# mikostrzewa/AprilSLAM

Measured on AMD Instinct MI355X. Metric: frames/sec at 1280x720, 20 tags/frame (detection + batched PnP), higher is better.
Workload: dtype u8/f64

## Files before the change

### aprilslam_amd/_lib.py

```python
import ctypes as C
import os

import numpy as np

_HERE = os.path.dirname(os.path.abspath(__file__))
LIB_PATH = os.environ.get("ASL_LIB") or os.path.join(_HERE, "libaprilslam.so")


class AslError(RuntimeError):
    pass


class AslDetection(C.Structure):
    _fields_ = [("id", C.c_int32), ("hamming", C.c_int32), ("margin", C.c_float), ("frame", C.c_int32),
                ("center", C.c_double * 2), ("corners", (C.c_double * 2) * 4)]


class AslPose(C.Structure):
    _fields_ = [("rvec", C.c_double * 3), ("tvec", C.c_double * 3), ("T", C.c_double * 16), ("ok", C.c_int32),
                ("reserved", C.c_int32)]


class AslMapTag(C.Structure):
    _fields_ = [("T", C.c_double * 12), ("valid", C.c_int32), ("reserved", C.c_int32)]
# ... 418 lines not shown
                                   corners.ctypes.data_as(dp), Kc.ctypes.data_as(dp), float(tag_size), int(fixed_tag),
                                   cam.ctypes.data_as(dp), tag.ctypes.data_as(dp), int(iters), stats.ctypes.data_as(dp)))
        return cam.reshape(-1, 4, 4), tag.reshape(-1, 4, 4), stats

    def debug_counters(self):
        buf = np.zeros(18, dtype=np.int64)
        n = C.c_size_t()
        check(self._L.asl_debug_fetch(self._h, 5, buf.ctypes.data, buf.nbytes, C.byref(n)))
        return buf

    def debug_image(self, what):
        c = self.debug_counters()
        B, sw, sh = int(c[0]), int(c[1]), int(c[2])
        dt = np.uint8 if what in (0, 1) else np.uint32
        buf = np.zeros((B, sh, sw), dtype=dt)
        n = C.c_size_t()
        check(self._L.asl_debug_fetch(self._h, what, buf.ctypes.data, buf.nbytes, C.byref(n)))
        return buf

    def debug_quads(self, cap=65536):
        buf = np.zeros(cap, dtype=QUAD_DTYPE)
        n = C.c_size_t()
        check(self._L.asl_debug_fetch(self._h, 4, buf.ctypes.data, buf.nbytes, C.byref(n)))
        return buf[:n.value]

    def debug_clusters(self):
        ncl = int(self.debug_counters()[3])
        buf = np.zeros((max(ncl, 1), 3), dtype=np.uint64)
        n = C.c_size_t()
        check(self._L.asl_debug_fetch(self._h, 6, buf.ctypes.data, buf.nbytes, C.byref(n)))
        return buf[:n.value]

    def debug_refit(self, reps):
        buf = np.zeros(7, dtype=np.int64)
        n = C.c_size_t()
        check(self._L.asl_debug_fetch(self._h, 7, buf.ctypes.data, int(reps), C.byref(n)))
        return buf

    def debug_division_check(self, exponent_limit=100):
        buf = np.zeros(2, dtype=np.int64)
        n = C.c_size_t()
        check(self._L.asl_debug_fetch(self._h, 8, buf.ctypes.data, int(exponent_limit), C.byref(n)))
        return int(buf[0]), int(buf[1])

    def phase_cycles(self, reset=True):
        buf = (C.c_uint64 * 64)()
        check(self._L.asl_debug_phase_cycles(self._h, buf, 1 if reset else 0))
        return np.array(list(buf), dtype=np.uint64)

    def set_profiling(self, on=True):
        check(self._L.asl_set_profiling(self._h, 1 if on else 0))

    def stage_times(self):
        names = (C.c_char_p * 32)()
        ms = (C.c_float * 32)()
        n = C.c_int()
        check(self._L.asl_stage_times(self._h, names, ms, 32, C.byref(n)))
        return {names[i].decode(): float(ms[i]) for i in range(n.value)}
```

### aprilslam_amd/csrc/aprilslam.hip

```cpp
#include "../../include/aprilslam.h"

#include <algorithm>
#include <chrono>
#include <cmath>
#include <cstdarg>
#include <cstdio>
#include <cstring>
#include <string>
#include <vector>

#include "asl_common.h"
#include "tag_standard41h12.inc"

#include "k_threshold.inc"
#include "k_cc.inc"
#include "k_cluster.inc"
#include "k_seg.inc"
#include "k_xchg.inc"
#include "k_quad.inc"
#include "k_decode.inc"
#include "k_pnp.inc"
#include "k_dedup.inc"
#include "k_graph.inc"
#include "k_render.inc"
// ... 181 lines not shown
    d->fam.width_at_border = kTag41h12WidthAtBorder;
    d->fam.total_width = kTag41h12TotalWidth;
    d->fam.reversed_border = 1;
    d->fam.ncodes = kTag41h12PinnedIds;
    for (int i = 0; i < kTag41h12NBits; i++) { d->fam.bit_x[i] = kTag41h12BitX[i]; d->fam.bit_y[i] = kTag41h12BitY[i]; }
    if (hipMalloc((void **)&d->d_codes, sizeof(unsigned long long) * kTag41h12NCodes) != hipSuccess) {
        delete d;
        return fail(ASL_ENOMEM, "hipMalloc(code book) failed");
    }
    if (hipMemcpy(d->d_codes, kTag41h12Codes, sizeof(unsigned long long) * kTag41h12NCodes, hipMemcpyHostToDevice) != hipSuccess) {
        (void)hipFree(d->d_codes);
        delete d;
        return fail(ASL_EDEVICE, "hipMemcpy(code book) failed");
    }
    d->fam.codes = d->d_codes;
    if (build_code_index(d)) {
        d->idx_start.release(); d->idx_entries.release();
        (void)hipFree(d->d_codes);
        delete d;
        return fail(ASL_ENOMEM, "code-book index allocation failed");
    }
    if (d->wtab.ensure(WEIGHT_TABLE_N)) {
        (void)hipFree(d->d_codes);
        delete d;
        return fail(ASL_ENOMEM, "hipMalloc(weight table) failed");
    }
    hipLaunchKernelGGL(k_weight_table, dim3((WEIGHT_TABLE_N + 255) / 256), dim3(256), 0, 0, d->wtab.p);
    if (hipDeviceSynchronize() != hipSuccess) {
        d->wtab.release();
        (void)hipFree(d->d_codes);
        delete d;
        return fail(ASL_EDEVICE, "weight table kernel failed");
    }
    (void)hipFuncSetAttribute(reinterpret_cast<const void *>(&k_fit_quads<256, true, CLASS3_CAP / 256>), hipFuncAttributeMaxDynamicSharedMemorySize, QUAD_LDS_BYTES(CLASS3_CAP));
    *out = d;
    return ASL_OK;
}

extern "C" void asl_detector_destroy(asl_detector *d)
{
    if (!d) return;
    (void)hipSetDevice(d->device);
    if (d->pending) (void)hipStreamSynchronize(d->p_stream);
    d->rootmask.release(); d->quad_list.release(); d->dense_tiles.release(); d->dense_seg.release(); d->seg_edges.release(); d->wmask.release(); d->bmask.release();
    d->dbg_thresh.release(); d->dbg_labels.release();
    d->frame_ndets.release(); d->frame_idx.release(); d->frame_nkeep.release(); d->frame_off.release(); d->out_det.release(); d->out_pose.release();
    if (d->host_pose) (void)hipHostFree(d->host_pose);
    if (d->host_nkeep) (void)hipHostFree(d->host_nkeep);
    d->in.release(); d->dgray.release(); d->tmin.release(); d->tmax.release(); d->tcut.release();
    d->parent.release(); d->sizes.release(); d->hkeys.release(); d->points.release(); d->hcounts.release(); d->class_lists.release(); d->stage_pos.release(); d->frame_cursor.release(); d->stage_rec.release();
    d->slot_cluster.release(); d->clusters.release(); d->quads.release(); d->scratch.release(); d->side_mom.release(); d->quadH.release(); d->wtab.release(); d->dets.release();
    d->counters.release(); d->pnp_corners.release(); d->pnp_out.release(); d->pnp_ok.release();
    d->gn.release();
    d->loc_obs.release(); d->loc_map.release(); d->loc_out.release();
    d->cal_ws.release(); d->cal_out.release();
    d->map_ws.release(); d->map_lm.release(); d->map_out.release();
    if (d->aux_stream) (void)hipStreamDestroy(d->aux_stream);
    if (d->copy_stream) (void)hipStreamDestroy(d->copy_stream);
    if (d->host_stream) (void)hipStreamDestroy(d->host_stream);
    for (hipEvent_t e : d->copy_done) (void)hipEventDestroy(e);
    if (d->d_codes) (void)hipFree(d->d_codes);
    d->idx_start.release(); d->idx_entries.release();
    if (d->host_det) (void)hipHostFree(d->host_det);
    if (d->pinned_counters) (void)hipHostFree(d->pinned_counters);
    for (int i = 0; i <= MAX_STAGES; i++) if (d->ev[i]) (void)hipEventDestroy(d->ev[i]);
    delete d;
}
// ... 111 lines not shown
    bad |= d->seg_edges.ensure(B * (size_t)seg_nwx(g) * (size_t)((g.sh + SEG_TH - 1) / SEG_TH));
    bad |= d->scratch.ensure((size_t)d->max_points * 8);
    bad |= d->dets.ensure(d->max_dets);
    bad |= d->frame_ndets.ensure(B);
    bad |= d->frame_nkeep.ensure(B);
    bad |= d->frame_off.ensure(B);
    bad |= d->frame_idx.ensure(B * (size_t)d->dets_per_frame);
    bad |= d->out_det.ensure(d->max_dets);
    bad |= d->out_pose.ensure(d->max_dets);
    bad |= d->counters.ensure(CNT__N);
    if (bad) return fail(ASL_ENOMEM, "device workspace allocation failed (%zu frames of %dx%d)", B, g.sw, g.sh);
    return ASL_OK;
}

#define STAGE(name)                                                        \
    do {                                                                   \
        if (d->profiling && d->nev < MAX_STAGES) {                         \
            d->stage_names[d->nev] = name;                                 \
            HIPCHK(hipEventRecord(d->ev[d->nev], st));                     \
            d->nev++;                                                      \
        }                                                                  \
    } while (0)

static void launch_fit_class(asl_detector *d, const Geom &g, int cls, unsigned int B, hipStream_t st)
{
    const int want_rev = d->fam.reversed_border ? 1 : 0, want_norm = d->fam.reversed_border ? 0 : 1;
    int tag_width = d->fam.width_at_border / g.f;
    if (tag_width < 3) tag_width = 3;
    const unsigned int qgrid = std::min<unsigned int>(d->max_clusters, std::max<unsigned int>(16384u, 32u * B));
    const unsigned int q2grid = std::min<unsigned int>(d->max_clusters, 2048u);
    const unsigned int *list = d->class_lists.p + (size_t)cls * d->max_clusters;
    switch (cls) {
    case 0:
        hipLaunchKernelGGL((k_fit_quads<64, true, CLASS0_CAP / 64>), dim3(qgrid), dim3(64), QUAD_LDS_BYTES(CLASS0_CAP), st, d->clusters.p, list, d->counters.p, 0,
                           d->max_clusters, CLASS0_CAP, d->points.p, d->dgray.p, g, tag_width, want_rev, want_norm, d->scratch.p, d->quads.p, d->wtab.p, d->side_mom.p);
        break;
    case 1:
        hipLaunchKernelGGL((k_fit_quads<128, true, CLASS1_CAP / 128>), dim3(qgrid), dim3(128), QUAD_LDS_BYTES(CLASS1_CAP), st, d->clusters.p, list, d->counters.p, 1,
                           d->max_clusters, CLASS1_CAP, d->points.p, d->dgray.p, g, tag_width, want_rev, want_norm, d->scratch.p, d->quads.p, d->wtab.p, d->side_mom.p);
        break;
    case 2:
        hipLaunchKernelGGL((k_fit_quads<256, true, CLASS2_CAP / 256>), dim3(q2grid), dim3(256), QUAD_LDS_BYTES(CLASS2_CAP), st, d->clusters.p, list, d->counters.p, 2,
                           d->max_clusters, CLASS2_CAP, d->points.p, d->dgray.p, g, tag_width, want_rev, want_norm, d->scratch.p, d->quads.p, d->wtab.p, d->side_mom.p);
        break;
    case 3:
        hipLaunchKernelGGL((k_fit_quads<256, true, CLASS3_CAP / 256>), dim3(q2grid), dim3(256), QUAD_LDS_BYTES(CLASS3_CAP), st, d->clusters.p, list, d->counters.p, 3,
                           d->max_clusters, CLASS3_CAP, d->points.p, d->dgray.p, g, tag_width, want_rev, want_norm, d->scratch.p, d->quads.p, d->wtab.p, d->side_mom.p);
        break;
    default:
        hipLaunchKernelGGL((k_fit_quads<256, false, 0>), dim3(q2grid), dim3(256), 0, st, d->clusters.p, list, d->counters.p, 4, d->max_clusters, 0, d->points.p,
                           d->dgray.p, g, tag_width, want_rev, want_norm, d->scratch.p, d->quads.p, d->wtab.p, d->side_mom.p);
        break;
    }
}

static void launch_quad_finish(asl_detector *d, const Geom &g, hipStream_t st)
{
    int tag_width = d->fam.width_at_border / g.f;
    if (tag_width < 3) tag_width = 3;
    hipLaunchKernelGGL(k_quad_finish, dim3(std::min<unsigned int>((d->max_clusters + 63) / 64, 4096u)), dim3(256), 0, st, d->quads.p, d->side_mom.p, d->counters.p,
                       d->max_clusters, tag_width);
}

static int enqueue_detect(asl_detector *d, const uint8_t *d_frames, const Geom &g, hipStream_t st, const CamDev *cam)
{
    dim3 blk(64, 4, 1);
    int thx = (g.sh + TILESZ - 1) / TILESZ;
    unsigned int B = (unsigned int)g.nframes;
    d->nev = 0;
    range_push("S0-S4 gray, decimate, threshold, segmentation, clusters");
    STAGE("k_hash_clear");
    hipLaunchKernelGGL(k_hash_clear, dim3((std::max<unsigned int>(d->nslots, std::max<unsigned int>(B, CNT__N)) + 255) / 256), dim3(256), 0, st, d->hkeys.p,
                       d->hcounts.p, d->nslots, d->counters.p, d->frame_cursor.p, d->frame_ndets.p, B);

    STAGE("k_decimate_minmax");
    if (g.f == 2) {
        const unsigned int ntile = (unsigned int)(g.tw * g.th);
        const unsigned int nrest = (unsigned int)(g.sw - 4 * g.tw) * (unsigned int)g.sh + (unsigned int)(g.sh - 4 * g.th) * (unsigned int)(4 * g.tw);
        if (ntile)
            hipLaunchKernelGGL((g.channels == 1 ? k_decimate2_tiles<1> : k_decimate2_tiles<3>), dim3((ntile + 255) / 256, B), dim3(256), 0, st, d_frames, g,
                               d->dgray.p, d->tmin.p, d->tmax.p);
        if (nrest)
            hipLaunchKernelGGL((g.channels == 1 ? k_decimate_rest<1> : k_decimate_rest<3>), dim3((nrest + 255) / 256, B), dim3(256), 0, st, d_frames, g,
// ... 14 lines not shown
        hipLaunchKernelGGL(k_seg_tile_dense, dim3(1024), dim3(64), 0, st, g, nwx, ntiles, d->wmask.p, d->bmask.p, d->parent.p, d->sizes.p,
                           d->rootmask.p, d->dense_seg.p, d->counters.p);
    }
    STAGE("k_seg_border");
    {
        const size_t nseams = nwx > 1 ? (size_t)B * g.sh * (nwx - 1) : 0;
        const unsigned int ncol_blocks = (unsigned int)((nseams + 63) / 64);
        const int nrb = (g.sh - 1) / SEG_TH;
        const unsigned int nrow_blocks = (unsigned int)nwx * (unsigned int)nrb * (unsigned int)B;
        if (ncol_blocks + nrow_blocks > 0)
            hipLaunchKernelGGL(k_seg_border, dim3(ncol_blocks + nrow_blocks), dim3(64), 0, st, d->wmask.p, d->bmask.p, d->seg_edges.p,
                               nwx * ((g.sh + SEG_TH - 1) / SEG_TH), g, nwx, d->parent.p, d->counters.p, ncol_blocks, nrb > 0 ? nrb : 1);
    }
    STAGE("k_seg_roots");
    hipLaunchKernelGGL(k_seg_roots, dim3((unsigned int)((nwords + 255) / 256)), dim3(256), 0, st, d->rootmask.p, g, nwx, d->parent.p, d->sizes.p);

    STAGE("k_seg_points");
    hipLaunchKernelGGL((k_seg_points<SEGP_PCAP, SEGP_RUNCAP, SEGP_NW, 1>), dim3(B, (nwx + SEGP_NW - 1) / SEGP_NW, pty), dim3(64 * SEGP_NW), 0, st,
                       d->wmask.p, d->bmask.p, g, nwx, d->parent.p, d->sizes.p, d->hkeys.p, d->hcounts.p, d->nslots - 1, d->stage_rec.p,
                       d->stage_pos.p, d->frame_cursor.p, d->stage_cap, d->dense_tiles.p, pty, d->counters.p);
    hipLaunchKernelGGL((k_seg_points<SEGP_PCAP_DENSE, SEGP_RUNCAP_DENSE, 1, 2>), dim3(256), dim3(64), 0, st, d->wmask.p, d->bmask.p, g, nwx,
                       d->parent.p, d->sizes.p, d->hkeys.p, d->hcounts.p, d->nslots - 1, d->stage_rec.p, d->stage_pos.p, d->frame_cursor.p,
                       d->stage_cap, d->dense_tiles.p, pty, d->counters.p);
    STAGE("k_cluster_filter");
    hipLaunchKernelGGL(k_cluster_filter, dim3((d->nslots + 1023) / 1024), dim3(1024), 0, st, d->hkeys.p, d->hcounts.p, d->nslots, g,
                       d->clusters.p, d->slot_cluster.p, d->class_lists.p, d->max_clusters, d->max_points, d->counters.p);
    STAGE("k_point_place");
    hipLaunchKernelGGL(k_point_place, dim3(16, B), dim3(256), 0, st, d->stage_rec.p, d->stage_pos.p, d->frame_cursor.p, d->stage_cap,
                       d->slot_cluster.p, d->points.p, d->counters.p);

    range_pop();
    range_push("S5 quad fit");
    for (int cls = 0; cls < NCLASSES; cls++) {
        static const char *const kFitStage[NCLASSES] = {"k_fit_quads<0>", "k_fit_quads<1>", "k_fit_quads<2>", "k_fit_quads<3>", "k_fit_quads<4>"};
        STAGE(kFitStage[cls]);
        launch_fit_class(d, g, cls, B, st);
    }

    STAGE("k_quad_finish");
    launch_quad_finish(d, g, st);
    range_pop();
    range_push("S6-S7 edge refinement, homography, decode");
    STAGE("k_quad_compact");
    hipLaunchKernelGGL(k_quad_compact, dim3((d->max_clusters + 1023) / 1024), dim3(1024), 0, st, d->quads.p, d->counters.p, d->max_clusters,
                       d->quad_list.p);
    unsigned int dgrid = std::min<unsigned int>(d->max_clusters, std::max<unsigned int>(8192u, 64u * B));
    STAGE("k_refine");
    hipLaunchKernelGGL((g.channels == 1 ? k_refine<1> : k_refine<3>), dim3(dgrid), dim3(64), 0, st, d->quads.p, d->counters.p, d->max_clusters, d_frames, g,
                       d->fam.reversed_border ? 1 : 0, d->refine, d->quadH.p, d->quad_list.p, d->side_mom.p);
    STAGE("k_homography");
    hipLaunchKernelGGL(k_homography, dim3(std::min<unsigned int>((d->max_clusters + 31) / 32, 2048u)), dim3(256), 0, st, d->quadH.p, d->counters.p, d->max_clusters,
                       d->quad_list.p, d->side_mom.p);
    STAGE("k_decode");
    hipLaunchKernelGGL((g.channels == 1 ? k_decode<1> : k_decode<3>), dim3(dgrid), dim3(64), 0, st, d->quads.p, d->quadH.p, d->counters.p, d->max_clusters, d_frames, g, d->fam,
                       d->maxhamming, d->dets.p, d->max_dets, d->counters.p, d->quad_list.p);

    range_pop();
    range_push("S9 PnP, S8 de-duplication");
    if (cam) {
        STAGE("k_pnp_dets");
        const int tpw = pnp_tpw(d->nd_guess ? d->nd_guess : (size_t)20 * B);
        hipLaunchKernelGGL(k_pnp_dets, dim3((d->max_dets + tpw - 1) / tpw), dim3(64), 0, st, d->dets.p, d->counters.p, d->max_dets, *cam, tpw);
    }
    STAGE("k_det_dedup");
    {
        const unsigned int cap_f = d->dets_per_frame;
        hipLaunchKernelGGL(k_det_bucket, dim3((d->max_dets + 255) / 256), dim3(256), 0, st, d->dets.p, d->counters.p, d->max_dets, d->frame_ndets.p,
// ... 669 lines not shown
        std::sort(cl.begin(), cl.end(), [](const ClusterRec &a, const ClusterRec &b) { return a.key < b.key; });
        unsigned long long *o = (unsigned long long *)dst;
        for (size_t i = 0; i < ncl; i++) {
            unsigned long long h = 0xcbf29ce484222325ull;
            if ((size_t)cl[i].offset + cl[i].count <= npts) {
                std::sort(pts.begin() + cl[i].offset, pts.begin() + cl[i].offset + cl[i].count);
                for (unsigned int k = 0; k < cl[i].count; k++) { h ^= pts[(size_t)cl[i].offset + k]; h *= 0x100000001b3ull; }
            }
            o[3 * i] = cl[i].key; o[3 * i + 1] = cl[i].count; o[3 * i + 2] = h;
        }
        *n_items = ncl;
        return ASL_OK;
    }
    case 7: {
        if (d->pending) return fail(ASL_EINVAL, "a batch is in flight on this detector");
        size_t ncl = (size_t)std::min<long long>(d->last_counters[CNT_NCLUSTERS], (long long)d->max_clusters);
        if (!ncl) return fail(ASL_EINVAL, "no clusters in the last batch");
        const size_t reps = bytes;
        std::vector<QuadRec> ref(ncl), cur(ncl);
        std::vector<ClusterRec> cl(ncl);
        HIPCHK(hipMemcpy(cl.data(), d->clusters.p, ncl * sizeof(ClusterRec), hipMemcpyDeviceToHost));
        long long *o = (long long *)dst;
        for (int k = 0; k < 2 + NCLASSES; k++) o[k] = 0;
        for (size_t r = 0; r < reps; r++) {
            for (int cls = 0; cls < NCLASSES - 1; cls++) launch_fit_class(d, g, cls, (unsigned int)g.nframes, nullptr);
            launch_quad_finish(d, g, nullptr);
            HIPCHK(hipGetLastError());
            HIPCHK(hipMemcpy((r ? cur : ref).data(), d->quads.p, ncl * sizeof(QuadRec), hipMemcpyDeviceToHost));
            if (!r) continue;
            for (size_t i = 0; i < ncl; i++) {
                const bool same = cur[i].valid == ref[i].valid && (!ref[i].valid || memcmp(cur[i].p, ref[i].p, sizeof ref[i].p) == 0);
                if (same) continue;
                const unsigned int cnt = cl[i].count;
                if (cnt > CLASS3_CAP) continue;
                o[1]++;
                o[2 + (cnt <= CLASS0_CAP ? 0 : (cnt <= CLASS1_CAP ? 1 : (cnt <= CLASS2_CAP ? 2 : (cnt <= CLASS3_CAP ? 3 : 4))))]++;
            }
        }
        o[0] = (long long)reps;
        *n_items = 2 + NCLASSES;
        return ASL_OK;
    }
    case 8: {
        unsigned long long *d_bad = nullptr, h_bad = 0;
        const int lim = bytes > 0 && bytes <= 900 ? (int)bytes : 100, blocks = 2048, per = 1024;
        HIPCHK(hipMalloc((void **)&d_bad, sizeof h_bad));
        HIPCHK(hipMemset(d_bad, 0, sizeof h_bad));
        hipLaunchKernelGGL(k_div_check, dim3(blocks), dim3(256), 0, nullptr, 20260301ull, per, lim, d_bad);
        hipError_t e8 = hipMemcpy(&h_bad, d_bad, sizeof h_bad, hipMemcpyDeviceToHost);
        (void)hipFree(d_bad);
        if (e8 != hipSuccess) return fail(ASL_EDEVICE, "division check failed: %s", hipGetErrorString(e8));
        ((long long *)dst)[0] = (long long)blocks * 256 * per;
        ((long long *)dst)[1] = (long long)h_bad;
        *n_items = 2;
        return ASL_OK;
    }
    default:
        return fail(ASL_EINVAL, "unknown debug item %d", what);
    }
}

extern "C" int asl_debug_phase_cycles(asl_detector *d, unsigned long long *out64, int reset)
{
    if (!d || !out64) return fail(ASL_EINVAL, "NULL argument");
    HIPCHK(hipSetDevice(d->device));
    std::vector<unsigned long long> all((size_t)64 * PHASE_SPREAD);
    HIPCHK(hipMemcpyFromSymbol(all.data(), HIP_SYMBOL(g_phase_cycles), sizeof(unsigned long long) * all.size()));
    for (int i = 0; i < 64; i++) {
        out64[i] = 0;
// ... 202 lines not shown
```

### aprilslam_amd/csrc/asl_common.h

```cpp
#pragma once
#include <hip/hip_runtime.h>
#include <stdint.h>

#define ASL_WAVE 64
#define TILESZ 4
#define MIN_WHITE_BLACK_DIFF 5
#define MIN_COMPONENT 25u
#define MAX_NMAXIMA 10
#define MAX_LINE_FIT_MSE 10.0
#define COS_CRITICAL_RAD 0.984807753012208
#define HASH_EMPTY 0xFFFFFFFFFFFFFFFFull
#define HASH_MAX_PROBE 512
#define NCLASSES 5
#define CLASS0_CAP 128
#define CLASS1_CAP 256
#define CLASS2_CAP 512
#define CLASS3_CAP 1024

template <typename T>
struct DevBuf {
    T *p = nullptr;
    size_t n = 0;
    int ensure(size_t want)
    {
        if (want <= n) return 0;
        if (p) { (void)hipFree(p); p = nullptr; n = 0; }
        hipError_t e = hipMalloc((void **)&p, want * sizeof(T));
        if (e != hipSuccess) { p = nullptr; return -1; }
        n = want;
        return 0;
    }
    void release() { if (p) (void)hipFree(p); p = nullptr; n = 0; }
};

struct Geom {
    int w, h;
    int stride;
    int channels;
    int f;
    int sw, sh;
    int tw, th;
    int nframes;
    size_t frame_pitch;
    size_t npix;
};

struct ClusterRec {
    uint64_t key;
    unsigned int offset;
    unsigned int count;
// ... 23 lines not shown
#define IDX_BUCKETS (1 << IDX_BUCKET_BITS)
#define IDX_MAX_CHUNKS 4
struct FamilyDev {
    int nbits, width_at_border, total_width, reversed_border, ncodes;
    int bit_x[64], bit_y[64];
    const unsigned long long *codes;
    int idx_nch;
    int idx_lo[IDX_MAX_CHUNKS], idx_w[IDX_MAX_CHUNKS];
    const unsigned short *idx_start;
    const unsigned long long *idx_entries;
};
__host__ __device__ __forceinline__ unsigned int idx_bucket(unsigned long long chunk_value, int width)
{
    return width <= IDX_BUCKET_BITS ? (unsigned int)chunk_value : (unsigned int)((chunk_value * 0x9E3779B97F4A7C15ull) >> (64 - IDX_BUCKET_BITS));
}

struct CamDev {
    double fx, fy, cx, cy, k1, k2, p1, p2, k3;
    double half;
    int both_minima;
    int pad;
};

enum {
    CNT_NCLUSTERS = 0,
    CNT_OVERFLOW_HASH = 1,
    CNT_OVERFLOW_POINTS = 2,
    CNT_OVERFLOW_CLUSTERS = 3,
    CNT_OVERFLOW_DETS = 4,
    CNT_UF_GUARD = 5,
    CNT_DEDUP_LIMIT = 6,
    CNT_NPOINTS = 16,
    CNT_CLASS0 = 32,
    CNT_NDETS = 112,
    CNT_NQUADS = 128,
    CNT_NKEEP = 144,
    CNT_DENSE_TILES = 160,
    CNT_DENSE_SEG = 161,
    CNT__N = 176
};
#define CNT_CLASS(c) (CNT_CLASS0 + 16 * (c))

struct Recip {
    double d, r;
};
__device__ __forceinline__ Recip recip_of(double d)
{
    double r = __builtin_amdgcn_rcp(d);
    double e = __builtin_fma(-d, r, 1.0);
    r = __builtin_fma(r, e, r);
    e = __builtin_fma(-d, r, 1.0);
    r = __builtin_fma(r, e, r);
    return Recip{d, r};
}
__device__ __forceinline__ double div_by(double a, const Recip &k)
{
    const double q = a * k.r;
    const double rem = __builtin_fma(-k.d, q, a);
    return __builtin_fma(rem, k.r, q);
}

__device__ __forceinline__ bool batch_poisoned(const long long *counters)
{
    return (counters[CNT_OVERFLOW_HASH] | counters[CNT_OVERFLOW_POINTS] | counters[CNT_OVERFLOW_CLUSTERS] | counters[CNT_OVERFLOW_DETS]) != 0;
}

#define PHASE_SPREAD 512
__device__ unsigned long long g_phase_cycles[64 * PHASE_SPREAD];
#ifdef ASL_PHASE_TIMING
#define PHASE_DECL()                                                                  \
    __shared__ unsigned long long ph_s__[16];                                         \
    long long ph_t__ = 0;                                                             \
// ... 58 lines not shown
```

### aprilslam_amd/csrc/k_cluster.inc

```

__device__ __forceinline__ unsigned long long hash64(unsigned long long k)
{
    k ^= k >> 33; k *= 0xff51afd7ed558ccdull;
    k ^= k >> 33; k *= 0xc4ceb9fe1a85ec53ull;
    k ^= k >> 33;
    return k;
}

__device__ __forceinline__ unsigned long long cluster_key(int fr, unsigned int a, unsigned int b)
{
    unsigned int hi = a > b ? a : b, lo = a > b ? b : a;
    return ((unsigned long long)fr << 48) | ((unsigned long long)hi << 24) | lo;
}

__device__ __noinline__ int hash_insert(unsigned long long *keys, unsigned int mask, unsigned long long key)
{
    unsigned int slot = (unsigned int)hash64(key) & mask;
#pragma unroll 1
    for (int probe = 0; probe < HASH_MAX_PROBE; probe++) {
        unsigned long long cur = __hip_atomic_load(&keys[slot], __ATOMIC_RELAXED, __HIP_MEMORY_SCOPE_AGENT);
        if (cur == key) return (int)slot;
        if (cur == HASH_EMPTY) {
            unsigned long long old = atomicCAS(&keys[slot], HASH_EMPTY, key);
            if (old == HASH_EMPTY || old == key) return (int)slot;
        }
        slot = (slot + 1) & mask;
    }
    return -1;
}

__global__ void __launch_bounds__(256) k_hash_clear(unsigned long long *keys, unsigned int *counts, unsigned int nslots, long long *counters,
                                                    unsigned int *frame_cursor, unsigned int *frame_ndets, unsigned int nframes)
{
    unsigned int i = blockIdx.x * blockDim.x + threadIdx.x;
    if (i < (unsigned int)CNT__N) counters[i] = 0;
    if (i < nframes) { frame_cursor[i] = 0u; frame_ndets[i] = 0u; }
    if (i >= nslots) return;
    keys[i] = HASH_EMPTY;
    counts[i] = 0;
}

#define POINT_BITS 36


__global__ void __launch_bounds__(1024) k_cluster_filter(const unsigned long long *__restrict__ keys, const unsigned int *__restrict__ counts,
                                                         unsigned int nslots, Geom g, ClusterRec *clusters, unsigned long long *slot_seg,
                                                         unsigned int *class_lists, unsigned int max_clusters, unsigned int max_points,
                                                         long long *counters)
{
    __shared__ unsigned int s_keep[16], s_pts[16], s_cls[16][NCLASSES];
    __shared__ unsigned long long s_base_ci, s_base_off, s_base_cls[NCLASSES];
    unsigned int i = blockIdx.x * blockDim.x + threadIdx.x;
    const int lane = threadIdx.x & 63, wid = threadIdx.x >> 6, nw = blockDim.x >> 6;
    unsigned long long key = i < nslots ? keys[i] : HASH_EMPTY;
    unsigned int cnt = i < nslots ? counts[i] : 0;
    bool keep = key != HASH_EMPTY && cnt >= 24u && cnt <= 3u * (unsigned int)(2 * g.sw + 2 * g.sh);
    int cls = cnt <= CLASS0_CAP ? 0 : (cnt <= CLASS1_CAP ? 1 : (cnt <= CLASS2_CAP ? 2 : (cnt <= CLASS3_CAP ? 3 : 4)));
    const unsigned long long lt = (1ull << lane) - 1ull;
    unsigned long long mask = __ballot(keep);
    unsigned int v = keep ? cnt : 0u, incl = v;
#pragma unroll
    for (int off = 1; off < 64; off <<= 1) {
        unsigned int o = __shfl_up(incl, off);
        if (lane >= off) incl += o;
    }
    unsigned long long mc[NCLASSES];
#pragma unroll
    for (int c = 0; c < NCLASSES; c++) mc[c] = __ballot(keep && cls == c);
    if (lane == 63) s_pts[wid] = incl;
    if (lane == 0) {
        s_keep[wid] = (unsigned int)__popcll(mask);
#pragma unroll
        for (int c = 0; c < NCLASSES; c++) s_cls[wid][c] = (unsigned int)__popcll(mc[c]);
    }
    __syncthreads();
    if (threadIdx.x == 0) {
        unsigned int tk = 0, tp = 0, tc[NCLASSES] = {0};
        for (int w = 0; w < nw; w++) {
            tk += s_keep[w]; tp += s_pts[w];
            for (int c = 0; c < NCLASSES; c++) tc[c] += s_cls[w][c];
        }
        s_base_ci = tk ? atomicAdd((unsigned long long *)&counters[CNT_NCLUSTERS], (unsigned long long)tk) : 0ull;
        s_base_off = tp ? atomicAdd((unsigned long long *)&counters[CNT_NPOINTS], (unsigned long long)tp) : 0ull;
        for (int c = 0; c < NCLASSES; c++)
            s_base_cls[c] = tc[c] ? atomicAdd((unsigned long long *)&counters[CNT_CLASS(c)], (unsigned long long)tc[c]) : 0ull;
    }
    __syncthreads();
    if (i < nslots) slot_seg[i] = ~0ull;
    if (!keep) return;
    unsigned long long ci = s_base_ci + __popcll(mask & lt), off = s_base_off + incl - v, cpos = s_base_cls[cls] + __popcll(mc[cls] & lt);
// ... 46 lines not shown
```

### aprilslam_amd/csrc/k_quad.inc

```

__device__ const unsigned int kCombo4of10[210] = {
    0x003210u, 0x014210u, 0x074310u, 0x1c4320u, 0x544321u, 0x025210u, 0x085310u, 0x1d5320u, 0x555321u, 0x0d5410u,
    0x225420u, 0x5a5421u, 0x315430u, 0x695431u, 0x8c5432u, 0x036210u, 0x096310u, 0x1e6320u, 0x566321u, 0x0e6410u,
    0x236420u, 0x5b6421u, 0x326430u, 0x6a6431u, 0x8d6432u, 0x126510u, 0x276520u, 0x5f6521u, 0x366530u, 0x6e6531u,
    0x916532u, 0x406540u, 0x786541u, 0x9b6542u, 0xaf6543u, 0x047210u, 0x0a7310u, 0x1f7320u, 0x577321u, 0x0f7410u,
    0x247420u, 0x5c7421u, 0x337430u, 0x6b7431u, 0x8e7432u, 0x137510u, 0x287520u, 0x607521u, 0x377530u, 0x6f7531u,
    0x927532u, 0x417540u, 0x797541u, 0x9c7542u, 0xb07543u, 0x167610u, 0x2b7620u, 0x637621u, 0x3a7630u, 0x727631u,
    0x957632u, 0x447640u, 0x7c7641u, 0x9f7642u, 0xb37643u, 0x4a7650u, 0x827651u, 0xa57652u, 0xb97653u, 0xc37654u,
    0x058210u, 0x0b8310u, 0x208320u, 0x588321u, 0x108410u, 0x258420u, 0x5d8421u, 0x348430u, 0x6c8431u, 0x8f8432u,
    0x148510u, 0x298520u, 0x618521u, 0x388530u, 0x708531u, 0x938532u, 0x428540u, 0x7a8541u, 0x9d8542u, 0xb18543u,
    0x178610u, 0x2c8620u, 0x648621u, 0x3b8630u, 0x738631u, 0x968632u, 0x458640u, 0x7d8641u, 0xa08642u, 0xb48643u,
    0x4b8650u, 0x838651u, 0xa68652u, 0xba8653u, 0xc48654u, 0x198710u, 0x2e8720u, 0x668721u, 0x3d8730u, 0x758731u,
    0x988732u, 0x478740u, 0x7f8741u, 0xa28742u, 0xb68743u, 0x4d8750u, 0x858751u, 0xa88752u, 0xbc8753u, 0xc68754u,
    0x508760u, 0x888761u, 0xab8762u, 0xbf8763u, 0xc98764u, 0xcd8765u, 0x069210u, 0x0c9310u, 0x219320u, 0x599321u,
    0x119410u, 0x269420u, 0x5e9421u, 0x359430u, 0x6d9431u, 0x909432u, 0x159510u, 0x2a9520u, 0x629521u, 0x399530u,
    0x719531u, 0x949532u, 0x439540u, 0x7b9541u, 0x9e9542u, 0xb29543u, 0x189610u, 0x2d9620u, 0x659621u, 0x3c9630u,
    0x749631u, 0x979632u, 0x469640u, 0x7e9641u, 0xa19642u, 0xb59643u, 0x4c9650u, 0x849651u, 0xa79652u, 0xbb9653u,
    0xc59654u, 0x1a9710u, 0x2f9720u, 0x679721u, 0x3e9730u, 0x769731u, 0x999732u, 0x489740u, 0x809741u, 0xa39742u,
    0xb79743u, 0x4e9750u, 0x869751u, 0xa99752u, 0xbd9753u, 0xc79754u, 0x519760u, 0x899761u, 0xac9762u, 0xc09763u,
    0xca9764u, 0xce9765u, 0x1b9810u, 0x309820u, 0x689821u, 0x3f9830u, 0x779831u, 0x9a9832u, 0x499840u, 0x819841u,
    0xa49842u, 0xb89843u, 0x4f9850u, 0x879851u, 0xaa9852u, 0xbe9853u, 0xc89854u, 0x529860u, 0x8a9861u, 0xad9862u,
    0xc19863u, 0xcb9864u, 0xcf9865u, 0x539870u, 0x8b9871u, 0xae9872u, 0xc29873u, 0xcc9874u, 0xd09875u, 0xd19876u,
};
__device__ const unsigned short kPairOff[12] = {0, 0, 0, 0, 0, 7, 20, 41, 72, 115, 172, 245};
__device__ const unsigned short kPairTab[245] = {
    0x0100, 0x0200, 0x0300, 0x0201, 0x0301, 0x0302, 0x0003, 0x0100, 0x0200, 0x0300, 0x0400, 0x0201, 0x0301, 0x0401,
    0x0302, 0x0402, 0x0403, 0x0003, 0x0004, 0x0104, 0x0100, 0x0200, 0x0300, 0x0400, 0x0500, 0x0201, 0x0301, 0x0401,
    0x0501, 0x0302, 0x0402, 0x0502, 0x0403, 0x0503, 0x0504, 0x0003, 0x0004, 0x0104, 0x0005, 0x0105, 0x0205, 0x0100,
    0x0200, 0x0300, 0x0400, 0x0500, 0x0600, 0x0201, 0x0301, 0x0401, 0x0501, 0x0601, 0x0302, 0x0402, 0x0502, 0x0602,
    0x0403, 0x0503, 0x0603, 0x0504, 0x0604, 0x0605, 0x0003, 0x0004, 0x0104, 0x0005, 0x0105, 0x0205, 0x0006, 0x0106,
    0x0206, 0x0306, 0x0100, 0x0200, 0x0300, 0x0400, 0x0500, 0x0600, 0x0700, 0x0201, 0x0301, 0x0401, 0x0501, 0x0601,
    0x0701, 0x0302, 0x0402, 0x0502, 0x0602, 0x0702, 0x0403, 0x0503, 0x0603, 0x0703, 0x0504, 0x0604, 0x0704, 0x0605,
    0x0705, 0x0706, 0x0003, 0x0004, 0x0104, 0x0005, 0x0105, 0x0205, 0x0006, 0x0106, 0x0206, 0x0306, 0x0007, 0x0107,
    0x0207, 0x0307, 0x0407, 0x0100, 0x0200, 0x0300, 0x0400, 0x0500, 0x0600, 0x0700, 0x0800, 0x0201, 0x0301, 0x0401,
    0x0501, 0x0601, 0x0701, 0x0801, 0x0302, 0x0402, 0x0502, 0x0602, 0x0702, 0x0802, 0x0403, 0x0503, 0x0603, 0x0703,
    0x0803, 0x0504, 0x0604, 0x0704, 0x0804, 0x0605, 0x0705, 0x0805, 0x0706, 0x0806, 0x0807, 0x0003, 0x0004, 0x0104,
    0x0005, 0x0105, 0x0205, 0x0006, 0x0106, 0x0206, 0x0306, 0x0007, 0x0107, 0x0207, 0x0307, 0x0407, 0x0008, 0x0108,
    0x0208, 0x0308, 0x0408, 0x0508, 0x0100, 0x0200, 0x0300, 0x0400, 0x0500, 0x0600, 0x0700, 0x0800, 0x0900, 0x0201,
    0x0301, 0x0401, 0x0501, 0x0601, 0x0701, 0x0801, 0x0901, 0x0302, 0x0402, 0x0502, 0x0602, 0x0702, 0x0802, 0x0902,
    0x0403, 0x0503, 0x0603, 0x0703, 0x0803, 0x0903, 0x0504, 0x0604, 0x0704, 0x0804, 0x0904, 0x0605, 0x0705, 0x0805,
    0x0905, 0x0706, 0x0806, 0x0906, 0x0807, 0x0907, 0x0908, 0x0003, 0x0004, 0x0104, 0x0005, 0x0105, 0x0205, 0x0006,
    0x0106, 0x0206, 0x0306, 0x0007, 0x0107, 0x0207, 0x0307, 0x0407, 0x0008, 0x0108, 0x0208, 0x0308, 0x0408, 0x0508,
    0x0009, 0x0109, 0x0209, 0x0309, 0x0409, 0x0509, 0x0609,
};

#define QUAD_LDS_PAD 2
#define QUAD_LDS_BYTES(cap) (64 * (cap) + 48 * QUAD_LDS_PAD)

struct Moments {
    const double *L[6];
    double tot[6];
    int sz;
};

#define WEIGHT_TABLE_N (2 * 255 * 255 + 1)
__global__ void __launch_bounds__(256) k_weight_table(double *__restrict__ t)
{
    const int n = blockIdx.x * blockDim.x + threadIdx.x;
    if (n < WEIGHT_TABLE_N) t[n] = sqrt((double)n) + 1;
}

__device__ __forceinline__ int fit_moments_dev(const Moments &m, int i0, int i1, double (&M)[6])
{
    const int sz = m.sz;
    const bool wrap = !(i0 < i1);
    const int N = wrap ? sz - i0 + i1 + 1 : i1 - i0 + 1;
    const bool sub = wrap || i0 > 0;
    const int ib = sub ? i0 - 1 : 0;
#pragma unroll
    for (int k = 0; k < 6; k++) {
        const double a = m.L[k][i1], b = sub ? m.L[k][ib] : 0.0, c = m.tot[k];
        const double plain = a - b, wrapped = (c - b) + a;
        M[k] = wrap ? wrapped : plain;
    }
    return N;
}

__device__ __forceinline__ void fit_line_moments_dev(const double (&M)[6], int N, double *lineparm, double *err, double *mse, bool normal = true)
{
    double Mx = M[0], My = M[1], Mxx = M[2], Mxy = M[3], Myy = M[4], W = M[5];
// ... 156 lines not shown
            if (e * NT < npad) {
                const unsigned long long other = lane_xor<J>(kr[e]);
                const bool keepmin = ((tid & J) == 0) == (((e * NT + tid) & K) == 0);
                kr[e] = ((kr[e] < other) == keepmin) ? kr[e] : other;
            }
        }
    }
    if constexpr (J > 1) bitonic_step<NT, PPT, K, J / 2>(kr, tid, npad, xk);
}

template <int NT, int PPT, int K>
__device__ __forceinline__ void bitonic_merge_stages(unsigned long long (&kr)[PPT], int tid, int npad, unsigned long long *xk)
{
    if (K <= npad) bitonic_step<NT, PPT, K, K / 2>(kr, tid, npad, xk);
    if constexpr (K < NT * PPT) bitonic_merge_stages<NT, PPT, 2 * K>(kr, tid, npad, xk);
}

template <int NT, bool LDS_ALL, int PPT>
__global__ void __launch_bounds__(NT) k_fit_quads(const ClusterRec *__restrict__ clusters, const unsigned int *__restrict__ class_list,
                                                  const long long *__restrict__ counters, int cls, unsigned int max_clusters, int cap,
                                                  unsigned long long *points, const uint8_t *__restrict__ dgray, Geom g, int tag_width,
                                                  int want_reversed, int want_normal, double *scratch, QuadRec *quads, const double *__restrict__ wtab,
                                                  double *__restrict__ side_mom)
{
    extern __shared__ __align__(16) unsigned char smem[];
    __shared__ int s_wave[4], s_base, s_n;
    __shared__ int s_maxidx[MAX_NMAXIMA], s_best[4];
    __shared__ double s_thresh;
    __shared__ double s_tmpd[4];
    __shared__ long long s_tmpl[4];
    __shared__ int s_tmpi[4];
    __shared__ double s_pnx[MAX_NMAXIMA * MAX_NMAXIMA], s_pny[MAX_NMAXIMA * MAX_NMAXIMA];
    __shared__ double s_pe_slab[LDS_ALL ? 1 : MAX_NMAXIMA * MAX_NMAXIMA], s_pm_slab[LDS_ALL ? 1 : MAX_NMAXIMA * MAX_NMAXIMA];
    double *const s_pe = LDS_ALL ? reinterpret_cast<double *>(smem) : s_pe_slab;
    double *const s_pm = LDS_ALL ? reinterpret_cast<double *>(smem) + MAX_NMAXIMA * MAX_NMAXIMA : s_pm_slab;
    const float LPF[7] = {0.011108996538242306f, 0.1353352832366127f, 0.6065306597126334f, 1.0f,
                          0.6065306597126334f, 0.1353352832366127f, 0.011108996538242306f};
    const int tid = threadIdx.x;
    PHASE_DECL();
    if (batch_poisoned(counters)) return;
    long long ncl64 = counters[CNT_CLASS(cls)];
    unsigned int ncl = ncl64 > (long long)max_clusters ? max_clusters : (unsigned int)ncl64;
    if (blockIdx.x >= ncl) return;

    constexpr int NREC = PPT > 0 ? PPT : 1;
    unsigned int ci_nx = 0, ci_nn = 0, ci_n3 = 0;
    ClusterRec cl_nx, cl_nn;
    unsigned long long recs_nx[NREC];
    if (PPT > 0) {
        const unsigned int G = gridDim.x, last = ncl - 1;
        ci_nx = class_list[blockIdx.x];
        ci_nn = class_list[min(blockIdx.x + G, last)];
        ci_n3 = class_list[min(blockIdx.x + 2 * G, last)];
        cl_nx = clusters[ci_nx];
        cl_nn = clusters[ci_nn];
#pragma unroll
        for (int e = 0; e < NREC; e++) {
            int i = tid + e * NT;
            recs_nx[e] = i < (int)cl_nx.count ? points[(size_t)cl_nx.offset + i] : 0ull;
        }
    }

    for (unsigned int li = blockIdx.x; li < ncl; li += gridDim.x) {
        __syncthreads();
        PHASE_INIT();
        unsigned int ci;
        ClusterRec cl;
        unsigned long long recs[NREC];
// ... 266 lines not shown
            int cand = (myerr == best && myerr < (double)HUGE_VALF) ? myrank : 0x7FFFFFFF;
            int brank = block_reduce<NT>(cand, 0x7FFFFFFF, s_tmpi, [](int a, int b) { return a < b ? a : b; });
            if (tid == 0) s_n = 0;
            __syncthreads();
            if (brank != 0x7FFFFFFF && cand == brank) {
                s_n = 1;
                for (int k = 0; k < 4; k++) s_best[k] = mine[k];
                s_thresh = best;
            }
            __syncthreads();
        }
        PHASE(7);
        if (!s_n) continue;
        if (!(s_thresh / sz < MAX_LINE_FIT_MSE)) continue;

        if (tid < 4) {
            int i0 = s_best[tid], i1 = s_best[(tid + 1) & 3];
            int len = i1 - i0;
            if (len < 0) len += sz;
            if (len > 8) {
                int t = len / 6;
                i0 = (i0 + t) % sz;
                i1 = (i1 + sz - t) % sz;
            }
            double M[6];
            fit_moments_dev(mom, i0, i1, M);
            double *out = side_mom + ((size_t)ci * 4 + tid) * 6;
#pragma unroll
            for (int k = 0; k < 6; k++) out[k] = M[k];
        }
        if (tid == 0) quads[ci].valid = 2;
        PHASE(8);
    }
    PHASE_FLUSH(0);
}

template <int CTRL>
__device__ __forceinline__ double quad_dpp(double v)
{
    const unsigned long long u = __builtin_bit_cast(unsigned long long, v);
    const unsigned int lo = (unsigned int)__builtin_amdgcn_update_dpp(0, (int)(unsigned int)u, CTRL, 0xf, 0xf, false);
    const unsigned int hi = (unsigned int)__builtin_amdgcn_update_dpp(0, (int)(unsigned int)(u >> 32), CTRL, 0xf, 0xf, false);
    return __builtin_bit_cast(double, ((unsigned long long)hi << 32) | lo);
}
#define QUAD_ROT1 0x39
#define QUAD_ROT2 0x4E
#define QUAD_ROT3 0x93

__global__ void __launch_bounds__(256) k_quad_finish(QuadRec *__restrict__ quads, const double *__restrict__ side_mom, const long long *__restrict__ counters,
                                                     unsigned int max_clusters, int tag_width)
{
    if (batch_poisoned(counters)) return;
    const long long ncl64 = counters[CNT_NCLUSTERS];
    const unsigned int ncl = ncl64 > (long long)max_clusters ? max_clusters : (unsigned int)ncl64;
    const int lane = threadIdx.x & 63, l = lane & 3;
    for (unsigned int c0 = blockIdx.x * 64u; c0 < ncl; c0 += gridDim.x * 64u) {
        const unsigned int ci = c0 + (threadIdx.x >> 2);
        const bool pending = ci < ncl && quads[ci].valid == 2;
        if (!__any(pending)) continue;
        double M[6];
        const double *in = side_mom + ((size_t)(pending ? ci : 0) * 4 + l) * 6;
#pragma unroll
        for (int k = 0; k < 6; k++) M[k] = pending ? in[k] : 1.0;
        double line[4], mse;
        fit_line_moments_dev(M, 0, line, nullptr, &mse);
        bool fail = mse > MAX_LINE_FIT_MSE;
        const double n0 = quad_dpp<QUAD_ROT1>(line[0]), n1 = quad_dpp<QUAD_ROT1>(line[1]), n2 = quad_dpp<QUAD_ROT1>(line[2]), n3 = quad_dpp<QUAD_ROT1>(line[3]);
// ... 62 lines not shown
```

Measured before the change: 366,700.

## Split quad-fit size classes finer and shrink block sizes for small clusters

Adds a sixth cluster size class (caps 64/128/256/512/1024) so small clusters run the fit_quads kernel with smaller workgroups (64 threads for the two smallest classes, 128 for the 256-cap class) and a larger grid. For very small caps, the pair-error scratch is placed in dynamic LDS after the point buffer, avoiding oversized static slabs. The goal is less idle-thread waste and better occupancy for the many small clusters, at the cost of one more kernel launch per frame and reshuffled counter offsets.

```diff
diff --git a/aprilslam_amd/_lib.py b/aprilslam_amd/_lib.py
--- a/aprilslam_amd/_lib.py
+++ b/aprilslam_amd/_lib.py
@@ -474,7 +474,7 @@
         return buf[:n.value]
 
     def debug_refit(self, reps):
-        buf = np.zeros(7, dtype=np.int64)
+        buf = np.zeros(8, dtype=np.int64)
         n = C.c_size_t()
         check(self._L.asl_debug_fetch(self._h, 7, buf.ctypes.data, int(reps), C.byref(n)))
         return buf
diff --git a/aprilslam_amd/csrc/aprilslam.hip b/aprilslam_amd/csrc/aprilslam.hip
--- a/aprilslam_amd/csrc/aprilslam.hip
+++ b/aprilslam_amd/csrc/aprilslam.hip
@@ -237,7 +237,7 @@
         delete d;
         return fail(ASL_EDEVICE, "weight table kernel failed");
     }
-    (void)hipFuncSetAttribute(reinterpret_cast<const void *>(&k_fit_quads<256, true, CLASS3_CAP / 256>), hipFuncAttributeMaxDynamicSharedMemorySize, QUAD_LDS_BYTES(CLASS3_CAP));
+    (void)hipFuncSetAttribute(reinterpret_cast<const void *>(&k_fit_quads<256, true, CLASS4_CAP / 256>), hipFuncAttributeMaxDynamicSharedMemorySize, QUAD_LDS_BYTES(CLASS4_CAP));
     *out = d;
     return ASL_OK;
 }
@@ -415,23 +415,27 @@
     const unsigned int *list = d->class_lists.p + (size_t)cls * d->max_clusters;
     switch (cls) {
     case 0:
-        hipLaunchKernelGGL((k_fit_quads<64, true, CLASS0_CAP / 64>), dim3(qgrid), dim3(64), QUAD_LDS_BYTES(CLASS0_CAP), st, d->clusters.p, list, d->counters.p, 0,
+        hipLaunchKernelGGL((k_fit_quads<64, true, CLASS0_CAP / 64>), dim3(qgrid), dim3(64), QUAD_LDS_BYTES_ALL(CLASS0_CAP), st, d->clusters.p, list, d->counters.p, 0,
                            d->max_clusters, CLASS0_CAP, d->points.p, d->dgray.p, g, tag_width, want_rev, want_norm, d->scratch.p, d->quads.p, d->wtab.p, d->side_mom.p);
         break;
     case 1:
-        hipLaunchKernelGGL((k_fit_quads<128, true, CLASS1_CAP / 128>), dim3(qgrid), dim3(128), QUAD_LDS_BYTES(CLASS1_CAP), st, d->clusters.p, list, d->counters.p, 1,
+        hipLaunchKernelGGL((k_fit_quads<64, true, CLASS1_CAP / 64>), dim3(qgrid), dim3(64), QUAD_LDS_BYTES_ALL(CLASS1_CAP), st, d->clusters.p, list, d->counters.p, 1,
                            d->max_clusters, CLASS1_CAP, d->points.p, d->dgray.p, g, tag_width, want_rev, want_norm, d->scratch.p, d->quads.p, d->wtab.p, d->side_mom.p);
         break;
     case 2:
-        hipLaunchKernelGGL((k_fit_quads<256, true, CLASS2_CAP / 256>), dim3(q2grid), dim3(256), QUAD_LDS_BYTES(CLASS2_CAP), st, d->clusters.p, list, d->counters.p, 2,
+        hipLaunchKernelGGL((k_fit_quads<128, true, CLASS2_CAP / 128>), dim3(qgrid), dim3(128), QUAD_LDS_BYTES(CLASS2_CAP), st, d->clusters.p, list, d->counters.p, 2,
                            d->max_clusters, CLASS2_CAP, d->points.p, d->dgray.p, g, tag_width, want_rev, want_norm, d->scratch.p, d->quads.p, d->wtab.p, d->side_mom.p);
         break;
     case 3:
         hipLaunchKernelGGL((k_fit_quads<256, true, CLASS3_CAP / 256>), dim3(q2grid), dim3(256), QUAD_LDS_BYTES(CLASS3_CAP), st, d->clusters.p, list, d->counters.p, 3,
                            d->max_clusters, CLASS3_CAP, d->points.p, d->dgray.p, g, tag_width, want_rev, want_norm, d->scratch.p, d->quads.p, d->wtab.p, d->side_mom.p);
         break;
+    case 4:
+        hipLaunchKernelGGL((k_fit_quads<256, true, CLASS4_CAP / 256>), dim3(q2grid), dim3(256), QUAD_LDS_BYTES(CLASS4_CAP), st, d->clusters.p, list, d->counters.p, 4,
+                           d->max_clusters, CLASS4_CAP, d->points.p, d->dgray.p, g, tag_width, want_rev, want_norm, d->scratch.p, d->quads.p, d->wtab.p, d->side_mom.p);
+        break;
     default:
-        hipLaunchKernelGGL((k_fit_quads<256, false, 0>), dim3(q2grid), dim3(256), 0, st, d->clusters.p, list, d->counters.p, 4, d->max_clusters, 0, d->points.p,
+        hipLaunchKernelGGL((k_fit_quads<256, false, 0>), dim3(q2grid), dim3(256), 0, st, d->clusters.p, list, d->counters.p, 5, d->max_clusters, 0, d->points.p,
                            d->dgray.p, g, tag_width, want_rev, want_norm, d->scratch.p, d->quads.p, d->wtab.p, d->side_mom.p);
         break;
     }
@@ -512,7 +516,7 @@
     range_pop();
     range_push("S5 quad fit");
     for (int cls = 0; cls < NCLASSES; cls++) {
-        static const char *const kFitStage[NCLASSES] = {"k_fit_quads<0>", "k_fit_quads<1>", "k_fit_quads<2>", "k_fit_quads<3>", "k_fit_quads<4>"};
+        static const char *const kFitStage[NCLASSES] = {"k_fit_quads<0>", "k_fit_quads<1>", "k_fit_quads<2>", "k_fit_quads<3>", "k_fit_quads<4>", "k_fit_quads<5>"};
         STAGE(kFitStage[cls]);
         launch_fit_class(d, g, cls, B, st);
     }
@@ -1248,9 +1252,9 @@
                 const bool same = cur[i].valid == ref[i].valid && (!ref[i].valid || memcmp(cur[i].p, ref[i].p, sizeof ref[i].p) == 0);
                 if (same) continue;
                 const unsigned int cnt = cl[i].count;
-                if (cnt > CLASS3_CAP) continue;
+                if (cnt > CLASS4_CAP) continue;
                 o[1]++;
-                o[2 + (cnt <= CLASS0_CAP ? 0 : (cnt <= CLASS1_CAP ? 1 : (cnt <= CLASS2_CAP ? 2 : (cnt <= CLASS3_CAP ? 3 : 4))))]++;
+                o[2 + fit_size_class(cnt)]++;
             }
         }
         o[0] = (long long)reps;
diff --git a/aprilslam_amd/csrc/asl_common.h b/aprilslam_amd/csrc/asl_common.h
--- a/aprilslam_amd/csrc/asl_common.h
+++ b/aprilslam_amd/csrc/asl_common.h
@@ -11,11 +11,16 @@
 #define COS_CRITICAL_RAD 0.984807753012208
 #define HASH_EMPTY 0xFFFFFFFFFFFFFFFFull
 #define HASH_MAX_PROBE 512
-#define NCLASSES 5
-#define CLASS0_CAP 128
-#define CLASS1_CAP 256
-#define CLASS2_CAP 512
-#define CLASS3_CAP 1024
+#define NCLASSES 6
+#define CLASS0_CAP 64
+#define CLASS1_CAP 128
+#define CLASS2_CAP 256
+#define CLASS3_CAP 512
+#define CLASS4_CAP 1024
+__host__ __device__ __forceinline__ int fit_size_class(unsigned int cnt)
+{
+    return cnt <= CLASS0_CAP ? 0 : (cnt <= CLASS1_CAP ? 1 : (cnt <= CLASS2_CAP ? 2 : (cnt <= CLASS3_CAP ? 3 : (cnt <= CLASS4_CAP ? 4 : 5))));
+}
 
 template <typename T>
 struct DevBuf {
@@ -105,12 +110,12 @@
     CNT_DEDUP_LIMIT = 6,
     CNT_NPOINTS = 16,
     CNT_CLASS0 = 32,
-    CNT_NDETS = 112,
-    CNT_NQUADS = 128,
-    CNT_NKEEP = 144,
-    CNT_DENSE_TILES = 160,
-    CNT_DENSE_SEG = 161,
-    CNT__N = 176
+    CNT_NDETS = 128,
+    CNT_NQUADS = 144,
+    CNT_NKEEP = 160,
+    CNT_DENSE_TILES = 176,
+    CNT_DENSE_SEG = 177,
+    CNT__N = 192
 };
 #define CNT_CLASS(c) (CNT_CLASS0 + 16 * (c))
 
diff --git a/aprilslam_amd/csrc/k_cluster.inc b/aprilslam_amd/csrc/k_cluster.inc
--- a/aprilslam_amd/csrc/k_cluster.inc
+++ b/aprilslam_amd/csrc/k_cluster.inc
@@ -55,7 +55,7 @@
     unsigned long long key = i < nslots ? keys[i] : HASH_EMPTY;
     unsigned int cnt = i < nslots ? counts[i] : 0;
     bool keep = key != HASH_EMPTY && cnt >= 24u && cnt <= 3u * (unsigned int)(2 * g.sw + 2 * g.sh);
-    int cls = cnt <= CLASS0_CAP ? 0 : (cnt <= CLASS1_CAP ? 1 : (cnt <= CLASS2_CAP ? 2 : (cnt <= CLASS3_CAP ? 3 : 4)));
+    const int cls = fit_size_class(cnt);
     const unsigned long long lt = (1ull << lane) - 1ull;
     unsigned long long mask = __ballot(keep);
     unsigned int v = keep ? cnt : 0u, incl = v;
diff --git a/aprilslam_amd/csrc/k_quad.inc b/aprilslam_amd/csrc/k_quad.inc
--- a/aprilslam_amd/csrc/k_quad.inc
+++ b/aprilslam_amd/csrc/k_quad.inc
@@ -44,8 +44,14 @@
     0x0009, 0x0109, 0x0209, 0x0309, 0x0409, 0x0509, 0x0609,
 };
 
+#ifndef ASL_PHASE_FIT_CLASS
+#define ASL_PHASE_FIT_CLASS -1
+#endif
+
 #define QUAD_LDS_PAD 2
 #define QUAD_LDS_BYTES(cap) (64 * (cap) + 48 * QUAD_LDS_PAD)
+#define QUAD_PAIR_BYTES (2 * MAX_NMAXIMA * MAX_NMAXIMA * 8)
+#define QUAD_LDS_BYTES_ALL(cap) (QUAD_LDS_BYTES(cap) + (16 * (cap) < QUAD_PAIR_BYTES ? QUAD_PAIR_BYTES : 0))
 
 struct Moments {
     const double *L[6];
@@ -268,8 +274,9 @@
     __shared__ int s_tmpi[4];
     __shared__ double s_pnx[MAX_NMAXIMA * MAX_NMAXIMA], s_pny[MAX_NMAXIMA * MAX_NMAXIMA];
     __shared__ double s_pe_slab[LDS_ALL ? 1 : MAX_NMAXIMA * MAX_NMAXIMA], s_pm_slab[LDS_ALL ? 1 : MAX_NMAXIMA * MAX_NMAXIMA];
-    double *const s_pe = LDS_ALL ? reinterpret_cast<double *>(smem) : s_pe_slab;
-    double *const s_pm = LDS_ALL ? reinterpret_cast<double *>(smem) + MAX_NMAXIMA * MAX_NMAXIMA : s_pm_slab;
+    constexpr int CAP = NT * PPT;
+    double *const s_pe = LDS_ALL ? reinterpret_cast<double *>(smem + (16 * CAP < QUAD_PAIR_BYTES ? QUAD_LDS_BYTES(CAP) : 0)) : s_pe_slab;
+    double *const s_pm = LDS_ALL ? s_pe + MAX_NMAXIMA * MAX_NMAXIMA : s_pm_slab;
     const float LPF[7] = {0.011108996538242306f, 0.1353352832366127f, 0.6065306597126334f, 1.0f,
                           0.6065306597126334f, 0.1353352832366127f, 0.011108996538242306f};
     const int tid = threadIdx.x;
@@ -602,7 +609,7 @@
         if (tid == 0) quads[ci].valid = 2;
         PHASE(8);
     }
-    PHASE_FLUSH(0);
+    if (ASL_PHASE_FIT_CLASS < 0 || cls == ASL_PHASE_FIT_CLASS) PHASE_FLUSH(0);
 }
 
 template <int CTRL>
```

New measurement: 366,800, median of 6. No clear change (+0.0%).
